# seryrzu/centroFlye

Hardware: NVIDIA B200
Metric: k-mer recruitment read-bases/s (higher is better)
Workload: dtype u64

## Files before the change

### centroflye_b200/csrc/cfk.cu

```cuda
#include <stdlib.h>
#include <string.h>

#include "cfk_common.cuh"

thread_local char cfk_g_err[512] = "";
long long cfk_g_launches = 0;

namespace {

using cfk::EMPTY;
using cfk::FULL;
using cfk::blocks_for;
using cfk::fail;
using cfk::home_slot;
using cfk::mix64;

__device__ __forceinline__ uint32_t base_at(const uint32_t* __restrict__ packed, int64_t pos) {
  return (__ldg(packed + (pos >> 4)) >> ((pos & 15) << 1)) & 3u;
}

__device__ __forceinline__ int64_t table_upsert(uint64_t* keys, int64_t cap, uint64_t key) {
  int64_t slot = home_slot(mix64(key), cap);
  for (int64_t probes = 0; probes < cap; ++probes) {
    uint64_t cur = ((volatile uint64_t*)keys)[slot];
// ... 1586 lines not shown
    if (incr_total) atomicAdd((unsigned long long*)(counters + 2), (unsigned long long)incr_total);
    if (splits) atomicAdd((unsigned long long*)(counters + 3), (unsigned long long)splits);
  }
}

struct JoinArgs {
  const int64_t* __restrict__ occ_ptr;
  const uint32_t* __restrict__ occ;
  const uint32_t* __restrict__ occ_last;
  const uint32_t* __restrict__ unit_last;
  uint32_t dmin, dmax, min_cov;
  double rel_threshold;
  uint4* edges;
  int64_t max_edges;
  uint8_t* selected;
  int64_t* edge_counter;
};

__device__ __forceinline__ uint32_t join_candidate(bool active, uint4 c, const JoinArgs& J) {
  constexpr uint32_t END = 0xFFFFFFFFu;
  uint32_t dmask = 0;
  uint32_t cnt0 = 0;
  uint64_t all_occ = 0;
  uint32_t ia = 0, ia_end = 0, ib0 = 0, ib_end = 0;
  if (active) {
    ia = (uint32_t)J.occ_ptr[c.x]; ia_end = (uint32_t)J.occ_ptr[c.x + 1];
    ib0 = (uint32_t)J.occ_ptr[c.y]; ib_end = (uint32_t)J.occ_ptr[c.y + 1];
    const uint32_t width = c.w - c.z;
    uint32_t ib = ib0;
    uint32_t bj = ib < ib_end ? __ldg(J.occ + ib) : END;
    for (uint32_t t = ia; t < ia_end; ++t) {
      const uint32_t g = __ldg(J.occ + t);
      const uint32_t rem = (J.occ_last ? __ldg(J.occ_last + t) : __ldg(J.unit_last + g)) - g;
      if (J.dmin > rem) continue;
      const uint32_t lo = g + J.dmin, hi = g + min(J.dmax, rem);
      while (bj < lo) {
        ++ib;
        bj = ib < ib_end ? __ldg(J.occ + ib) : END;
      }
      uint32_t jj = ib, v = bj;
      while (v <= hi) {
        ++all_occ;
        const uint32_t dj = (v - g) - c.z;
        if (dj <= width) dmask |= 1u << dj;
        cnt0 += dj == 0u;
        ++jj;
        v = jj < ib_end ? __ldg(J.occ + jj) : END;
      }
    }
  }
  uint32_t n_cand_d = 0;
  while (__any_sync(FULL, dmask != 0)) {
    bool keep = false;
    uint32_t d = 0, cnt = 0;
    if (dmask) {
      const uint32_t dj = (uint32_t)(__ffs(dmask) - 1);
      d = c.z + dj;
      dmask &= dmask - 1;
      if (dj == 0u) {
        cnt = cnt0;
      } else {
        uint32_t ib = ib0;
        uint32_t bj = ib < ib_end ? __ldg(J.occ + ib) : END;
        for (uint32_t t = ia; t < ia_end; ++t) {
          const uint32_t g = __ldg(J.occ + t);
          const uint32_t rem = (J.occ_last ? __ldg(J.occ_last + t) : __ldg(J.unit_last + g)) - g;
          if (d > rem) continue;
          const uint32_t want = g + d;
          while (bj < want) {
            ++ib;
            bj = ib < ib_end ? __ldg(J.occ + ib) : END;
          }
          cnt += bj == want;
        }
      }
      if (cnt >= J.min_cov) {
        ++n_cand_d;
        keep = ((double)cnt / (double)all_occ) >= J.rel_threshold;
      }
    }
    const int64_t pos = warp_append(keep, J.edge_counter);
    if (keep) {
      if (pos < J.max_edges) J.edges[pos] = make_uint4(c.x, c.y, d, cnt);
      J.selected[c.x] = 1;
      J.selected[c.y] = 1;
    }
  }
  return n_cand_d;
}

constexpr int SK_BITS = CFK_SKETCH_BITS;
constexpr int SK_TBL_BYTES = 1 << SK_BITS;
constexpr uint32_t SK_OFF_MASK = 0x3FFFu;
constexpr uint32_t SK_DUP = 0x8000u;
constexpr uint32_t SK_NULL = SK_DUP | (uint32_t)SK_TBL_BYTES;
constexpr int SK_PAD_BYTES = 128;
constexpr int SK_L2_SLOTS = 256;
constexpr int SK_L2_MAX = 192;
constexpr int SK_Q_SLOTS = 256;
constexpr int SK_WINDOW = 128;
constexpr int SK_WARP_BYTES = SK_TBL_BYTES + SK_PAD_BYTES + SK_L2_SLOTS * 4 + SK_Q_SLOTS * 4;
constexpr int SK_WARPS_FIT = (227 * 1024 - 256) / SK_WARP_BYTES;
constexpr int SK_WARPS = SK_WARPS_FIT > 32 ? 32 : SK_WARPS_FIT;
constexpr uint32_t SK_CAP = (uint32_t)SK_TBL_BYTES / CFK_SKETCH_LOAD_DIV;
constexpr int SK_ND_MAX = 16;
static_assert(SK_BITS >= 10 && SK_BITS <= 13, "codes are 16 bit: offset in bits 0..13 (the null byte sits at 2^SK_BITS), bit 15 = no store");
static_assert(SK_WARPS >= 1, "sketch does not fit shared memory");

__host__ __device__ __forceinline__ int64_t sk_block(int64_t first_entry, int64_t unit) { return (first_entry >> 7) + unit; }
static_assert(SK_WINDOW == 128, "sk_block shifts by 7");

__device__ __forceinline__ uint32_t sk_hash(uint32_t id) { return (id * 0x9E3779B1u) >> (32 - SK_BITS); }

__device__ __forceinline__ uint32_t lds_u8(uint32_t a) {
  uint32_t v;
  asm volatile("ld.shared.u8 %0, [%1];" : "=r"(v) : "r"(a) : "memory");
  return v;
}
__device__ __forceinline__ void sts_u8(uint32_t a, uint32_t v) { asm volatile("st.shared.u8 [%0], %1;" ::"r"(a), "r"(v) : "memory"); }
__device__ __forceinline__ uint32_t atom_cas_shared(uint32_t a, uint32_t cmp, uint32_t val) {
  uint32_t old;
  asm volatile("atom.shared.cas.b32 %0, [%1], %2, %3;" : "=r"(old) : "r"(a), "r"(cmp), "r"(val) : "memory");
  return old;
}

__global__ void __launch_bounds__(256) sketch_codes_kernel(const int64_t* __restrict__ unit_ptr, const uint32_t* __restrict__ ids,
                                                           int64_t n_units, uint2* __restrict__ codes) {
  __shared__ uint32_t bm[8][SK_TBL_BYTES / 32];
  const int lane = threadIdx.x & 31, warp = threadIdx.x >> 5;
  const int64_t u = (int64_t)blockIdx.x * 8 + warp;
  if (u >= n_units) return;
  const int64_t b = unit_ptr[u], e = unit_ptr[u + 1];
  if (b == e) return;
  for (int i = lane; i < SK_TBL_BYTES / 32; i += 32) bm[warp][i] = 0;
  __syncwarp();
  uint2* out = codes + sk_block(b, u) * 32 + lane;
  for (int64_t p0 = b; p0 < e; p0 += SK_WINDOW, out += 32) {
    uint32_t c[4];
#pragma unroll
    for (int j = 0; j < 4; ++j) {
      const int64_t p = p0 + 32 * j + lane;
      c[j] = SK_NULL;
      if (p < e) {
        const uint32_t h = sk_hash(ids[p]);
        const uint32_t old = atomicOr(&bm[warp][h >> 5], 1u << (h & 31u));
        c[j] = h | (((old >> (h & 31u)) & 1u) ? SK_DUP : 0u);
      }
    }
    *out = make_uint2(c[0] | (c[1] << 16), c[2] | (c[3] << 16));
  }
}

__global__ void __launch_bounds__(256) sketch_codes_banked_kernel(const int64_t* __restrict__ unit_ptr,
                                                                  const uint32_t* __restrict__ ids, int64_t n_units,
                                                                  uint2* __restrict__ codes, uint4* __restrict__ perm_ids) {
  __shared__ uint32_t bm[8][SK_TBL_BYTES / 32];
  __shared__ int s_cnt[8][32];
  __shared__ int s_nover[8];
  __shared__ uint16_t s_code[8][SK_WINDOW], s_ocode[8][SK_WINDOW];
  __shared__ uint32_t s_id[8][SK_WINDOW], s_oid[8][SK_WINDOW];
  __shared__ uint8_t s_free[8][SK_WINDOW];
  const int lane = threadIdx.x & 31, warp = threadIdx.x >> 5;
  const uint32_t lt = (1u << lane) - 1u;
  const int64_t u = (int64_t)blockIdx.x * 8 + warp;
  if (u >= n_units) return;
  const int64_t b = unit_ptr[u], e = unit_ptr[u + 1];
  if (b == e) return;
  for (int i = lane; i < SK_TBL_BYTES / 32; i += 32) bm[warp][i] = 0;
  __syncwarp();
  int64_t blk = sk_block(b, u);
  for (int64_t p0 = b; p0 < e; p0 += SK_WINDOW, ++blk) {
    const int n = (int)min((int64_t)SK_WINDOW, e - p0), rows = (n + 31) >> 5;
    s_cnt[warp][lane] = 0;
    if (lane == 0) s_nover[warp] = 0;
#pragma unroll
    for (int j = 0; j < 4; ++j) {
      s_code[warp][4 * lane + j] = (uint16_t)(SK_DUP | (uint32_t)(SK_TBL_BYTES + 4 * lane));
      s_id[warp][4 * lane + j] = 0u;
    }
    __syncwarp();
#pragma unroll
    for (int j = 0; j < 4; ++j) {
      const int q = 32 * j + lane;
      if (q < n) {
        const uint32_t id = ids[p0 + q];
        const uint32_t h = sk_hash(id);
        const uint32_t old = atomicOr(&bm[warp][h >> 5], 1u << (h & 31u));
        const uint16_t code = (uint16_t)(h | (((old >> (h & 31u)) & 1u) ? SK_DUP : 0u));
        const int bank = (int)((h >> 2) & 31u);
        const int r = atomicAdd(&s_cnt[warp][bank], 1);
        if (r < rows) {
          s_code[warp][4 * bank + r] = code;
          s_id[warp][4 * bank + r] = id;
        } else {
          const int o = atomicAdd(&s_nover[warp], 1);
          s_ocode[warp][o] = code;
          s_oid[warp][o] = id;
        }
      }
    }
    __syncwarp();
    const int mine = min(s_cnt[warp][lane], rows);
    int base = 0;
    for (int r = rows - 1; r >= 0; --r) {
      const bool fr = mine <= r;
      const unsigned bal = __ballot_sync(FULL, fr);
      if (fr) s_free[warp][base + __popc(bal & lt)] = (uint8_t)(4 * lane + r);
      base += __popc(bal);
    }
    __syncwarp();
    const int nover = s_nover[warp];
    for (int o = lane; o < nover; o += 32) {
      const int slot = s_free[warp][o];
      s_code[warp][slot] = s_ocode[warp][o];
      s_id[warp][slot] = s_oid[warp][o];
    }
    __syncwarp();
    const uint32_t c0 = s_code[warp][4 * lane], c1 = s_code[warp][4 * lane + 1], c2 = s_code[warp][4 * lane + 2],
                   c3 = s_code[warp][4 * lane + 3];
    codes[blk * 32 + lane] = make_uint2(c0 | (c1 << 16), c2 | (c3 << 16));
    perm_ids[blk * 32 + lane] = make_uint4(s_id[warp][4 * lane], s_id[warp][4 * lane + 1], s_id[warp][4 * lane + 2],
                                           s_id[warp][4 * lane + 3]);
    __syncwarp();
  }
}

struct SketchArgs {
  const int64_t* __restrict__ unit_ptr;
  const uint32_t* __restrict__ ids;
  bool banked;
  const uint2* __restrict__ codes;
  const uint32_t* __restrict__ unit_last;
  const uint32_t* __restrict__ last_a;
  const uint32_t* __restrict__ occ_a;
  int64_t m;
  int64_t n_kmers;
  uint32_t a;
  uint32_t thr;
  uint4* cand;
  int64_t max_cand;
  int64_t* counters;
  struct SketchChunk* chunk;
  bool prefetch;
};

constexpr int SK_CAND_CHUNK = 256;
constexpr uint32_t SK_NO_CAND = 0xFFFFFFFFu;
struct SketchChunk {
  int64_t pos, end, emitted;
};

__device__ __forceinline__ void sk_close_chunk(const SketchArgs& A) {
  const int lane = threadIdx.x & 31;
  for (int64_t q = A.chunk->pos + lane; q < A.chunk->end; q += 32)
    if (q < A.max_cand) A.cand[q] = make_uint4(SK_NO_CAND, 0u, 0u, 0u);
  A.chunk->pos = A.chunk->end;
}

__device__ bool sk_drain(uint32_t l2base, uint32_t qbase, const SketchArgs& A, int qn, int64_t lo_id, int64_t hi_id,
                         int& claims) {
  const int lane = threadIdx.x & 31;
  bool ovf = false;
  __syncwarp();
  for (int base = 0; base < qn; base += 32) {
    const int idx = base + lane;
    if (idx < qn) {
      const uint32_t pos = lds<uint32_t>(qbase + (uint32_t)idx * 4u);
      const uint32_t b = __ldg(A.ids + pos);
      if (b != A.a && (int64_t)b >= lo_id && (int64_t)b < hi_id) {
        const uint32_t key = b + 1u;
        uint32_t slot = (b * 0x85EBCA77u) >> 24;
        static_assert(SK_L2_SLOTS == 256, "slot hash takes the top 8 bits");
        int probes = 0;
        for (; probes < SK_L2_SLOTS; ++probes) {
          const uint32_t old = atom_cas_shared(l2base + slot * 4u, 0u, key);
          if (old == 0u) { ++claims; break; }
          if (old == key) break;
          slot = (slot + 1u) & (uint32_t)(SK_L2_SLOTS - 1);
        }
        if (probes == SK_L2_SLOTS) ovf = true;
      }
    }
  }
  __syncwarp();
  const int total = __reduce_add_sync(FULL, claims);
  return !(__any_sync(FULL, ovf) || total > SK_L2_MAX);
}

struct SketchPre {
  uint32_t up, ue;
  int64_t unit;
};

__device__ __forceinline__ void sk_prefetch_unit(const uint2* codes, uint32_t up, uint32_t ue, uint32_t ub) {
  if (ue <= up) return;
  const uint32_t n_blocks = (ue - up + (uint32_t)SK_WINDOW - 1u) / (uint32_t)SK_WINDOW;
  const char* base = reinterpret_cast<const char*>(codes + (size_t)ub * 32u);
  for (uint32_t b = 0; b < n_blocks && b < 4u; ++b) {
    asm volatile("prefetch.global.L2 [%0];" ::"l"(base + b * 256u));
    asm volatile("prefetch.global.L2 [%0];" ::"l"(base + b * 256u + 128u));
  }
}

__device__ int sketch_pass(uint32_t tbase, const SketchArgs& A, int d0, int nd, int64_t lo_id, int64_t hi_id,
                           const SketchPre* pre = nullptr) {
  const int lane = threadIdx.x & 31;
  const uint32_t lt = (1u << lane) - 1u;
  const uint32_t l2base = tbase + SK_TBL_BYTES + SK_PAD_BYTES, qbase = l2base + SK_L2_SLOTS * 4;
  const uint32_t thr = A.thr;
  uint32_t up = 0, ue = 0, ub = 0;
  unsigned rest = 0;
  int src = 0;
  uint32_t p = 0, e = 0, cb = 0;
  uint2 w = make_uint2(0, 0);
  if (pre != nullptr) {
    up = pre->up;
    ue = pre->ue;
    ub = (uint32_t)sk_block((int64_t)up, pre->unit);
    if (A.prefetch) sk_prefetch_unit(A.codes, up, ue, ub);
    rest = __ballot_sync(FULL, ue > up);
    if (rest) {
      src = __ffs(rest) - 1;
      rest &= rest - 1;
      p = __shfl_sync(FULL, up, src); e = __shfl_sync(FULL, ue, src); cb = __shfl_sync(FULL, ub, src);
      w = __ldg(A.codes + (size_t)cb * 32u + lane);
    }
  }
#pragma unroll 4
  for (int i = lane; i < (SK_TBL_BYTES + SK_PAD_BYTES + SK_L2_SLOTS * 4) / 16; i += 32)
    sts128(tbase + (uint32_t)i * 16u, make_uint4(0, 0, 0, 0));
  __syncwarp();
  int qn = 0, claims = 0;
  const int64_t n_items = A.m * (int64_t)nd;
  for (int64_t i0 = 0; i0 < n_items; i0 += 32) {
    if (pre != nullptr) {
      if (e <= p) continue;
    } else {
      const int64_t it = i0 + lane;
      up = 0; ue = 0; ub = 0;
      if (it < n_items) {
        const int64_t t = (nd == 1) ? it : it / nd;
        const int64_t g = (int64_t)__ldg(A.occ_a + t);
        const int64_t u = g + d0 + (it - t * nd);
        if (u <= last_unit_of(A.unit_last, A.last_a, t, g)) {
          const int64_t p0 = __ldg(A.unit_ptr + u);
          up = (uint32_t)p0;
          ue = (uint32_t)__ldg(A.unit_ptr + u + 1);
          ub = (uint32_t)sk_block(p0, u);
        }
      }
      if (A.prefetch) sk_prefetch_unit(A.codes, up, ue, ub);
      rest = __ballot_sync(FULL, ue > up);
      if (!rest) continue;
      src = __ffs(rest) - 1;
      rest &= rest - 1;
      p = __shfl_sync(FULL, up, src); e = __shfl_sync(FULL, ue, src); cb = __shfl_sync(FULL, ub, src);
      w = __ldg(A.codes + (size_t)cb * 32u + lane);
    }
    for (;;) {
      uint32_t np = p + SK_WINDOW, ne = e, ncb = cb + 1u;
      const bool sw = np >= ne;
      const int nsrc = (__ffs(rest) - 1) & 31;
      const uint32_t sp = __shfl_sync(FULL, up, nsrc), se = __shfl_sync(FULL, ue, nsrc), sb = __shfl_sync(FULL, ub, nsrc);
      const bool more = !sw || rest != 0u;
      np = sw ? sp : np;
      ne = sw ? se : ne;
      ncb = sw ? sb : ncb;
      rest = sw ? (rest & (rest - 1u)) : rest;
      uint2 nw = make_uint2(0, 0);
      if (more) nw = __ldg(A.codes + (size_t)ncb * 32u + lane);
      const uint32_t a0 = tbase + (w.x & SK_OFF_MASK), a1 = tbase + ((w.x >> 16) & SK_OFF_MASK);
      const uint32_t a2 = tbase + (w.y & SK_OFF_MASK), a3 = tbase + ((w.y >> 16) & SK_OFF_MASK);
      const uint32_t o0 = lds_u8(a0), o1 = lds_u8(a1), o2 = lds_u8(a2), o3 = lds_u8(a3);
      if (!(w.x & SK_DUP)) sts_u8(a0, min(o0 + 1u, 255u));
      if ((int32_t)w.x >= 0) sts_u8(a1, min(o1 + 1u, 255u));
      if (!(w.y & SK_DUP)) sts_u8(a2, min(o2 + 1u, 255u));
      if ((int32_t)w.y >= 0) sts_u8(a3, min(o3 + 1u, 255u));
      if (__any_sync(FULL, max(max(o0, o1), max(o2, o3)) >= thr)) {
        const bool hs[4] = {o0 >= thr, o1 >= thr, o2 >= thr, o3 >= thr};
#pragma unroll
        for (int i = 0; i < 4; ++i) {
          const unsigned bal = __ballot_sync(FULL, hs[i]);
          if (hs[i]) sts(qbase + (uint32_t)(qn + __popc(bal & lt)) * 4u, A.banked ? (cb << 7) + 4u * (uint32_t)lane + (uint32_t)i : p + (uint32_t)lane + 32u * i);
          qn += __popc(bal);
        }
        if (qn > SK_Q_SLOTS - SK_WINDOW) {
          if (!sk_drain(l2base, qbase, A, qn, lo_id, hi_id, claims)) return -1;
          qn = 0;
        }
      }
      __syncwarp();
      if (!more) break;
      p = np; e = ne; cb = ncb; w = nw;
    }
  }
  if (!sk_drain(l2base, qbase, A, qn, lo_id, hi_id, claims)) return -1;
  int emitted = 0;
  for (int i = lane; i < SK_L2_SLOTS / 4; i += 32) {
    const uint4 q = lds128(l2base + (uint32_t)i * 16u);
    const uint32_t w[4] = {q.x, q.y, q.z, q.w};
    if (__any_sync(FULL, (q.x | q.y | q.z | q.w) != 0u)) {
#pragma unroll
      for (int j = 0; j < 4; ++j) {
        const bool take = w[j] != 0u;
        const unsigned bal = __ballot_sync(FULL, take);
        if (bal) {
          const int n = __popc(bal);
          if (A.chunk->pos + n > A.chunk->end) {
            sk_close_chunk(A);
            unsigned long long base = 0;
            if (lane == 0) base = atomicAdd((unsigned long long*)A.counters, (unsigned long long)SK_CAND_CHUNK);
            base = __shfl_sync(FULL, base, 0);
            A.chunk->pos = (int64_t)base;
            A.chunk->end = (int64_t)base + SK_CAND_CHUNK;
          }
          const int64_t pos = A.chunk->pos + __popc(bal & lt);
          if (take && pos < A.max_cand) A.cand[pos] = make_uint4(A.a, w[j] - 1u, (uint32_t)d0, (uint32_t)(d0 + nd - 1));
          A.chunk->pos += n;
          A.chunk->emitted += n;
        }
        emitted += take;
      }
    }
  }
  __syncwarp();
  return emitted;
}

__device__ void sketch_source(uint32_t tbase, const SketchArgs& A, int dmin, int dlim, int64_t& splits) {
  const int lane = threadIdx.x & 31;
  int d0 = dmin;
  int nd_force = SK_ND_MAX;
  const bool cached = A.m <= 32;
  int64_t cg = 0, clim = 0;
  uint32_t W0 = 0, W1 = 0, W2 = 0, W3 = 0, W4 = 0;
  auto window_at = [&](int d) -> uint32_t { return lane < A.m ? (uint32_t)__ldg(A.unit_ptr + min(cg + d, clim)) : 0u; };
  if (cached) {
    if (lane < A.m) {
      cg = (int64_t)__ldg(A.occ_a + lane);
      clim = last_unit_of(A.unit_last, A.last_a, lane, cg) + 1;
    }
    W0 = window_at(d0); W1 = window_at(d0 + 1); W2 = window_at(d0 + 2); W3 = window_at(d0 + 3); W4 = window_at(d0 + 4);
  }
  auto advance_d = [&](int by) {
    for (int i = 0; i < by; ++i) {
      ++d0;
      if (cached) {
        W0 = W1; W1 = W2; W2 = W3; W3 = W4;
        W4 = window_at(d0 + 4);
      }
    }
  };
  while (d0 <= dlim) {
    const int nd_max = min(nd_force, dlim - d0 + 1);
    int nd = 0;
    uint32_t tot = 0, first = 0;
    bool stop = false;
    for (int jb = 0; jb < nd_max && !stop; jb += 4) {
      uint32_t c0 = 0, c1 = 0, c2 = 0, c3 = 0;
      if (cached && jb == 0) {
        c0 = W1 - W0; c1 = W2 - W1; c2 = W3 - W2; c3 = W4 - W3;
      } else
      for (int64_t t0 = 0; t0 < A.m; t0 += 32) {
        const int64_t t = t0 + lane;
        if (t < A.m) {
          const int64_t g = (int64_t)__ldg(A.occ_a + t);
          const int64_t lim = last_unit_of(A.unit_last, A.last_a, t, g) + 1;
          const int64_t u = g + d0 + jb;
          const uint32_t p0 = (uint32_t)__ldg(A.unit_ptr + min(u, lim)), p1 = (uint32_t)__ldg(A.unit_ptr + min(u + 1, lim)),
                         p2 = (uint32_t)__ldg(A.unit_ptr + min(u + 2, lim)), p3 = (uint32_t)__ldg(A.unit_ptr + min(u + 3, lim)),
                         p4 = (uint32_t)__ldg(A.unit_ptr + min(u + 4, lim));
          c0 += p1 - p0; c1 += p2 - p1; c2 += p3 - p2; c3 += p4 - p3;
        }
      }
      const uint32_t c[4] = {__reduce_add_sync(FULL, c0), __reduce_add_sync(FULL, c1), __reduce_add_sync(FULL, c2),
                             __reduce_add_sync(FULL, c3)};
      if (jb == 0) first = c[0];
#pragma unroll
      for (int k = 0; k < 4; ++k) {
        if (stop || jb + k >= nd_max) { stop = true; continue; }
        if (c[k] <= SK_CAP && tot <= SK_CAP - c[k]) { tot += c[k]; ++nd; } else stop = true;
      }
    }
    if (nd < 1) { nd = 1; tot = first; }
    if (tot == 0) { advance_d(nd); nd_force = SK_ND_MAX; continue; }
    bool redo = false;
    int64_t lo_id = 0, width = A.n_kmers;
    const SketchPre pre{W0, W1, cg + d0};
    const SketchPre* prep = (cached && nd == 1) ? &pre : nullptr;
    while (lo_id < A.n_kmers) {
      const int64_t hi_id = min(A.n_kmers, lo_id + width);
      const int emitted = sketch_pass(tbase, A, d0, nd, lo_id, hi_id, prep);
      if (emitted < 0) {
        ++splits;
        if (nd > 1) { nd_force = nd >> 1; redo = true; break; }
        width = max((int64_t)1, (hi_id - lo_id) >> 1);
        continue;
      }
      lo_id = hi_id;
      if (emitted < SK_L2_MAX / 2 && width < A.n_kmers) width <<= 1;
    }
    if (redo) continue;
    advance_d(nd);
    nd_force = SK_ND_MAX;
  }
}

__global__ void __launch_bounds__(SK_WARPS * 32, 1)
pair_sketch_kernel(const int64_t* __restrict__ unit_ptr, const uint32_t* __restrict__ ids, const uint2* __restrict__ codes,
                   const uint32_t* __restrict__ perm_ids, const uint32_t* __restrict__ unit_last, const int64_t* __restrict__ occ_ptr,
                   const uint32_t* __restrict__ occ, const uint32_t* __restrict__ occ_last, int64_t n_kmers, int64_t a_begin,
                   int64_t a_end, int32_t a_stride, int32_t min_d, int32_t max_d, uint32_t min_cov, uint4* cand,
                   int64_t max_cand, int64_t* counters, int prefetch) {
  extern __shared__ __align__(16) unsigned char pc_smem[];
  const int lane = threadIdx.x & 31, warp = threadIdx.x >> 5;
  const uint32_t tbase = (uint32_t)__cvta_generic_to_shared(pc_smem) + (uint32_t)warp * SK_WARP_BYTES;
  const int dmin = max(min_d, 1);
  int64_t incr_total = 0, splits = 0;
  SketchChunk chunk{0, 0, 0};
  for (;;) {
    unsigned long long item = 0;
    if (lane == 0) item = atomicAdd((unsigned long long*)(counters + 1), 1ull);
    item = __shfl_sync(FULL, item, 0);
    const int64_t a64 = a_begin + (int64_t)item * a_stride;
    if (a64 >= a_end) break;
    const uint32_t a = (uint32_t)a64;
    const int64_t o0 = occ_ptr[a], m = occ_ptr[a + 1] - o0;
    if (m == 0) continue;
    const uint32_t* occ_a = occ + o0;
    const uint32_t* last_a = occ_last ? occ_last + o0 : nullptr;
    const int dlim = source_scope(unit_ptr, unit_last, occ_a, m, dmin, max_d, min_cov, incr_total, last_a);
    if (dlim < dmin) continue;
    SketchArgs A{unit_ptr, perm_ids ? perm_ids : ids, perm_ids != nullptr, codes, unit_last, last_a, occ_a, m, n_kmers, a, min_cov - 1u, cand,
                 max_cand, counters, &chunk, prefetch != 0};
    sketch_source(tbase, A, dmin, dlim, splits);
  }
  {
    SketchArgs A{};
    A.cand = cand;
    A.max_cand = max_cand;
    A.chunk = &chunk;
    sk_close_chunk(A);
  }
  if (lane == 0) {
    if (chunk.emitted) atomicAdd((unsigned long long*)(counters + 4), (unsigned long long)chunk.emitted);
    if (incr_total) atomicAdd((unsigned long long*)(counters + 2), (unsigned long long)incr_total);
    if (splits) atomicAdd((unsigned long long*)(counters + 3), (unsigned long long)splits);
  }
}

__global__ void pair_join_kernel(const uint4* __restrict__ cand, int64_t n_cand, const int64_t* __restrict__ occ_ptr,
                                 const uint32_t* __restrict__ occ, const uint32_t* __restrict__ occ_last,
                                 const uint32_t* __restrict__ unit_last, int32_t min_d, int32_t max_d, uint32_t min_cov,
                                 double rel_threshold, uint4* edges, int64_t max_edges, uint8_t* selected, int64_t* counters) {
  const int64_t i = (int64_t)blockIdx.x * blockDim.x + threadIdx.x;
  const JoinArgs J{occ_ptr, occ, occ_last, unit_last, (uint32_t)max(min_d, 1), (uint32_t)max(max_d, 0), min_cov, rel_threshold,
                   edges, max_edges, selected, counters};
  uint4 c = make_uint4(0xFFFFFFFFu, 0, 0, 0);
  if (i < n_cand) c = cand[i];
  uint32_t n_cand_d = join_candidate(c.x != 0xFFFFFFFFu, c, J);
  for (int o = 16; o >= 1; o >>= 1) n_cand_d += __shfl_xor_sync(FULL, n_cand_d, o);
  if ((threadIdx.x & 31) == 0 && n_cand_d) atomicAdd((unsigned long long*)(counters + 2), (unsigned long long)n_cand_d);
}

__global__ void flag_indices_kernel(const uint8_t* __restrict__ flags, int64_t n, uint32_t* out, int64_t* counters) {
  const int64_t i = (int64_t)blockIdx.x * blockDim.x + threadIdx.x;
  bool take = i < n && flags[i] != 0;
  int64_t pos = warp_append(take, counters);
  if (take) out[pos] = (uint32_t)i;
}


}

extern "C" {

int cfk_abi_version(void) { return 1; }
const char* cfk_last_error(void) { return cfk_g_err; }
int cfk_pair_table_bytes_per_warp(void) { return PC_TBL_BYTES; }
int cfk_pair_warps_per_block(void) { return PC_WARPS; }
int64_t cfk_launch_count(void) { return (int64_t)__atomic_load_n(&cfk_g_launches, __ATOMIC_RELAXED); }

int cfk_table_init(uint64_t* table, int64_t cap, cfk_stream_t stream) {
  if (cap < 1) return fail(CFK_ERR_INVALID, "cfk_table_init: cap < 1");
  table_init_kernel<<<(unsigned)blocks_for(cap, 256), 256, 0, (cudaStream_t)stream>>>(table, cap);
  CFK_CHECK_LAUNCH("table_init_kernel", 1);
  return CFK_OK;
}

int cfk_docfreq_count(const uint32_t* packed, const int64_t* read_off, const int64_t* read_len, const int32_t* order,
                      int64_t n_reads, int k, uint64_t* table, int64_t cap, int64_t* counters, int32_t n_blocks,
                      cfk_stream_t stream) {
  if (k < 1 || k > 31) return fail(CFK_ERR_INVALID, "cfk_docfreq_count: k must be in [1, 31]");
  if (cap < 1 || n_reads < 0 || n_blocks < 1) return fail(CFK_ERR_INVALID, "cfk_docfreq_count: bad sizes");
  if (n_reads == 0) return CFK_OK;
  static unsigned long long attr_done = 0;
  const int smem = (DF_SET_SLOTS + DF_TILE_WORDS) * 4;
  {
    cudaError_t e = cfk::ensure_dynamic_smem(docfreq_kernel, smem, &attr_done);
    if (e != cudaSuccess) return fail(CFK_ERR_CUDA, "cfk_docfreq_count: cudaFuncSetAttribute", e);
  }
  docfreq_kernel<<<(unsigned)n_blocks, DF_THREADS, smem, (cudaStream_t)stream>>>(packed, read_off, read_len, order, n_reads,
                                                                               k, table, cap, counters);
  CFK_CHECK_LAUNCH("docfreq_kernel", 1);
  return CFK_OK;
}

int cfk_docfreq_plan(const int64_t* read_len, const int32_t* order, int64_t n_reads, int k, int32_t* n_pass,
                     cfk_stream_t stream) {
  if (k < 1 || k > 31) return fail(CFK_ERR_INVALID, "cfk_docfreq_plan: k must be in [1, 31]");
  if (n_reads < 0) return fail(CFK_ERR_INVALID, "cfk_docfreq_plan: bad sizes");
  if (n_reads == 0) return CFK_OK;
  docfreq_plan_kernel<<<(unsigned)blocks_for(n_reads, 256), 256, 0, (cudaStream_t)stream>>>(read_len, order, n_reads, k, n_pass);
  CFK_CHECK_LAUNCH("docfreq_plan_kernel", 1);
  return CFK_OK;
}

int cfk_docfreq_count_resident(const uint32_t* packed, const int64_t* read_off, const int64_t* read_len,
                               const int32_t* order, const int64_t* item_ptr, int64_t n_reads, int k, uint64_t* table,
                               int64_t cap, int64_t* counters, int32_t n_blocks, cfk_stream_t stream) {
  if (k < 1 || k > 31) return fail(CFK_ERR_INVALID, "cfk_docfreq_count_resident: k must be in [1, 31]");
  if (cap < 1 || n_reads < 0 || n_blocks < 1) return fail(CFK_ERR_INVALID, "cfk_docfreq_count_resident: bad sizes");
  if (n_reads == 0) return CFK_OK;
  static unsigned long long attr_done = 0;
  const int smem = DF3_SMEM_WORDS * 4;
  {
    cudaError_t e = cfk::ensure_dynamic_smem(docfreq_resident_kernel, smem, &attr_done);
    if (e != cudaSuccess) return fail(CFK_ERR_CUDA, "cfk_docfreq_count_resident: cudaFuncSetAttribute", e);
  }
  docfreq_resident_kernel<<<(unsigned)n_blocks * DF3_BLOCKS_PER_SM, DF3_THREADS, smem, (cudaStream_t)stream>>>(
      packed, read_off, read_len, order, item_ptr, n_reads, k, table, cap, counters);
  CFK_CHECK_LAUNCH("docfreq_resident_kernel", 1);
  return CFK_OK;
}

int cfk_kmer_count_total(const uint32_t* packed, const int64_t* read_off, const int64_t* read_len, const int32_t* tile_read,
                         const int64_t* tile_start, int64_t n_tiles, int k, uint64_t* table, int64_t cap, int64_t* counters,
                         cfk_stream_t stream) {
  if (k < 1 || k > 31) return fail(CFK_ERR_INVALID, "cfk_kmer_count_total: k must be in [1, 31]");
  if (cap < 1 || n_tiles < 0 || n_tiles >= (1ll << 31)) return fail(CFK_ERR_INVALID, "cfk_kmer_count_total: bad sizes");
  if (n_tiles == 0) return CFK_OK;
  kmer_count_kernel<false><<<(unsigned)n_tiles, KC_THREADS, 0, (cudaStream_t)stream>>>(packed, read_off, read_len, tile_read,
                                                                                     tile_start, k, table, cap, counters);
  CFK_CHECK_LAUNCH("kmer_count_kernel", 1);
  return CFK_OK;
}

int cfk_kmer_count_canonical(const uint32_t* packed, const int64_t* read_off, const int64_t* read_len, const int32_t* tile_read,
                             const int64_t* tile_start, int64_t n_tiles, int k, uint64_t* table, int64_t cap,
                             int64_t* counters, cfk_stream_t stream) {
  if (k < 1 || k > 31) return fail(CFK_ERR_INVALID, "cfk_kmer_count_canonical: k must be in [1, 31]");
  if (cap < 1 || n_tiles < 0 || n_tiles >= (1ll << 31)) return fail(CFK_ERR_INVALID, "cfk_kmer_count_canonical: bad sizes");
  if (n_tiles == 0) return CFK_OK;
  kmer_count_kernel<true><<<(unsigned)n_tiles, KC_THREADS, 0, (cudaStream_t)stream>>>(packed, read_off, read_len, tile_read,
                                                                                    tile_start, k, table, cap, counters);
  CFK_CHECK_LAUNCH("kmer_count_kernel", 1);
  return CFK_OK;
}

int cfk_kmer_count_tile(void) { return KC_TILE; }

int cfk_kmer_position_keys(const uint32_t* packed, int64_t n_bases, int k, int pos_bits, uint64_t* keys, cfk_stream_t stream) {
  if (k < 1 || k > 31) return fail(CFK_ERR_INVALID, "cfk_kmer_position_keys: k must be in [1, 31]");
  if (pos_bits < 1 || 2 * k + pos_bits > 63 || n_bases < 0 || n_bases >= (1ll << pos_bits) || n_bases >= (1ll << 32))
    return fail(CFK_ERR_INVALID, "cfk_kmer_position_keys: need n_bases < 2^pos_bits and 2k + pos_bits <= 63");
  const int64_t n = n_bases - k + 1;
  if (n <= 0) return CFK_OK;
  kmer_position_keys_kernel<<<(unsigned)blocks_for(n, 256), 256, 0, (cudaStream_t)stream>>>(packed, n, k, pos_bits, keys);
  CFK_CHECK_LAUNCH("kmer_position_keys_kernel", 1);
  return CFK_OK;
}

int cfk_adjacent_gaps(const uint64_t* keys, int64_t n, int pos_bits, uint32_t* gaps, cfk_stream_t stream) {
  if (n < 0 || pos_bits < 1 || pos_bits > 62) return fail(CFK_ERR_INVALID, "cfk_adjacent_gaps: bad sizes");
  if (n == 0) return CFK_OK;
  adjacent_gaps_kernel<<<(unsigned)blocks_for(n, 256), 256, 0, (cudaStream_t)stream>>>(keys, n, pos_bits, gaps);
  CFK_CHECK_LAUNCH("adjacent_gaps_kernel", 1);
  return CFK_OK;
}

int cfk_table_merge(const uint64_t* keys, const uint32_t* nreads, const uint32_t* nmulti, int64_t n, uint64_t* table,
                    int64_t cap, int64_t* counters, cfk_stream_t stream) {
  if (n < 0 || cap < 1) return fail(CFK_ERR_INVALID, "cfk_table_merge: bad sizes");
  if (n == 0) return CFK_OK;
  table_merge_kernel<<<(unsigned)blocks_for(n, 256), 256, 0, (cudaStream_t)stream>>>(keys, nreads, nmulti, n, table, cap,
                                                                                      counters);
  CFK_CHECK_LAUNCH("table_merge_kernel", 1);
  return CFK_OK;
}

int cfk_table_lookup(const uint64_t* table, int64_t cap, const uint64_t* keys, int64_t n, uint32_t* out_nreads,
                     uint32_t* out_nmulti, cfk_stream_t stream) {
  if (n < 0 || cap < 1) return fail(CFK_ERR_INVALID, "cfk_table_lookup: bad sizes");
  if (n == 0) return CFK_OK;
  table_lookup_kernel<<<(unsigned)blocks_for(n, 256), 256, 0, (cudaStream_t)stream>>>(table, cap, keys, n, out_nreads, out_nmulti);
  CFK_CHECK_LAUNCH("table_lookup_kernel", 1);
// ... 327 lines not shown
```

Before: 5.805 billion.

## Restructure sketch pass to process per-unit row counts with tail-specialized code

The sketch inner loop now tracks, for each unit, how many 32-position rows remain instead of a start/end pair. Full 4-row blocks go through a tight loop that prefetches the next block, and a final partial block is handled by templated variants that touch only 1–3 rows. This removes shared-memory loads, stores and threshold ballots for rows past the unit end, along with the per-iteration shuffles of end positions. The cost is more branching and code size, plus a serial dependent load inside the inner loop.

```diff
diff --git a/centroflye_b200/csrc/cfk.cu b/centroflye_b200/csrc/cfk.cu
--- a/centroflye_b200/csrc/cfk.cu
+++ b/centroflye_b200/csrc/cfk.cu
@@ -1912,28 +1912,65 @@
   }
 }
 
+template <int K>
+__device__ __forceinline__ bool sk_rows(uint2 w, uint32_t pos0, uint32_t tbase, uint32_t qbase, uint32_t l2base,
+                                        const SketchArgs& A, int64_t lo_id, int64_t hi_id, int& qn, int& claims) {
+  const int lane = threadIdx.x & 31;
+  const uint32_t c[4] = {w.x & 0xFFFFu, w.x >> 16, w.y & 0xFFFFu, w.y >> 16};
+  uint32_t a[K], o[K];
+#pragma unroll
+  for (int i = 0; i < K; ++i) {
+    a[i] = tbase + (c[i] & SK_OFF_MASK);
+    o[i] = lds_u8(a[i]);
+  }
+#pragma unroll
+  for (int i = 0; i < K; ++i)
+    if (!(c[i] & SK_DUP)) sts_u8(a[i], min(o[i] + 1u, 255u));
+  uint32_t mx = o[0];
+#pragma unroll
+  for (int i = 1; i < K; ++i) mx = max(mx, o[i]);
+  if (__any_sync(FULL, mx >= A.thr)) {
+    const uint32_t lt = (1u << lane) - 1u;
+    const uint32_t step = A.banked ? 1u : 32u;
+#pragma unroll
+    for (int i = 0; i < K; ++i) {
+      const bool hs = o[i] >= A.thr;
+      const unsigned bal = __ballot_sync(FULL, hs);
+      if (hs) sts(qbase + (uint32_t)(qn + __popc(bal & lt)) * 4u, pos0 + step * (uint32_t)i);
+      qn += __popc(bal);
+    }
+    if (qn > SK_Q_SLOTS - SK_WINDOW) {
+      if (!sk_drain(l2base, qbase, A, qn, lo_id, hi_id, claims)) return false;
+      qn = 0;
+    }
+  }
+  return true;
+}
+
 __device__ int sketch_pass(uint32_t tbase, const SketchArgs& A, int d0, int nd, int64_t lo_id, int64_t hi_id,
                            const SketchPre* pre = nullptr) {
   const int lane = threadIdx.x & 31;
   const uint32_t lt = (1u << lane) - 1u;
   const uint32_t l2base = tbase + SK_TBL_BYTES + SK_PAD_BYTES, qbase = l2base + SK_L2_SLOTS * 4;
-  const uint32_t thr = A.thr;
-  uint32_t up = 0, ue = 0, ub = 0;
+  const uint2* codes = A.codes + lane;
+  uint32_t up = 0, ur = 0, ub = 0;
   unsigned rest = 0;
   int src = 0;
-  uint32_t p = 0, e = 0, cb = 0;
+  uint32_t p = 0, cb = 0, R = 0;
   uint2 w = make_uint2(0, 0);
   if (pre != nullptr) {
     up = pre->up;
-    ue = pre->ue;
+    ur = (pre->ue - up + 31u) >> 5;
     ub = (uint32_t)sk_block((int64_t)up, pre->unit);
-    if (A.prefetch) sk_prefetch_unit(A.codes, up, ue, ub);
-    rest = __ballot_sync(FULL, ue > up);
+    if (A.prefetch) sk_prefetch_unit(A.codes, up, pre->ue, ub);
+    rest = __ballot_sync(FULL, ur != 0u);
     if (rest) {
       src = __ffs(rest) - 1;
       rest &= rest - 1;
-      p = __shfl_sync(FULL, up, src); e = __shfl_sync(FULL, ue, src); cb = __shfl_sync(FULL, ub, src);
-      w = __ldg(A.codes + (size_t)cb * 32u + lane);
+      p = __shfl_sync(FULL, up, src);
+      R = __shfl_sync(FULL, ur, src);
+      cb = __shfl_sync(FULL, ub, src);
+      w = __ldg(codes + (size_t)cb * 32u);
     }
   }
 #pragma unroll 4
@@ -1944,10 +1981,11 @@
   const int64_t n_items = A.m * (int64_t)nd;
   for (int64_t i0 = 0; i0 < n_items; i0 += 32) {
     if (pre != nullptr) {
-      if (e <= p) continue;
+      if (R == 0u) continue;
     } else {
       const int64_t it = i0 + lane;
-      up = 0; ue = 0; ub = 0;
+      uint32_t ue = 0;
+      up = 0; ub = 0;
       if (it < n_items) {
         const int64_t t = (nd == 1) ? it : it / nd;
         const int64_t g = (int64_t)__ldg(A.occ_a + t);
@@ -1960,48 +1998,41 @@
         }
       }
       if (A.prefetch) sk_prefetch_unit(A.codes, up, ue, ub);
-      rest = __ballot_sync(FULL, ue > up);
+      ur = (ue - up + 31u) >> 5;
+      rest = __ballot_sync(FULL, ur != 0u);
       if (!rest) continue;
       src = __ffs(rest) - 1;
       rest &= rest - 1;
-      p = __shfl_sync(FULL, up, src); e = __shfl_sync(FULL, ue, src); cb = __shfl_sync(FULL, ub, src);
-      w = __ldg(A.codes + (size_t)cb * 32u + lane);
+      p = __shfl_sync(FULL, up, src);
+      R = __shfl_sync(FULL, ur, src);
+      cb = __shfl_sync(FULL, ub, src);
+      w = __ldg(codes + (size_t)cb * 32u);
     }
     for (;;) {
-      uint32_t np = p + SK_WINDOW, ne = e, ncb = cb + 1u;
-      const bool sw = np >= ne;
       const int nsrc = (__ffs(rest) - 1) & 31;
-      const uint32_t sp = __shfl_sync(FULL, up, nsrc), se = __shfl_sync(FULL, ue, nsrc), sb = __shfl_sync(FULL, ub, nsrc);
-      const bool more = !sw || rest != 0u;
-      np = sw ? sp : np;
-      ne = sw ? se : ne;
-      ncb = sw ? sb : ncb;
-      rest = sw ? (rest & (rest - 1u)) : rest;
-      uint2 nw = make_uint2(0, 0);
-      if (more) nw = __ldg(A.codes + (size_t)ncb * 32u + lane);
-      const uint32_t a0 = tbase + (w.x & SK_OFF_MASK), a1 = tbase + ((w.x >> 16) & SK_OFF_MASK);
-      const uint32_t a2 = tbase + (w.y & SK_OFF_MASK), a3 = tbase + ((w.y >> 16) & SK_OFF_MASK);
-      const uint32_t o0 = lds_u8(a0), o1 = lds_u8(a1), o2 = lds_u8(a2), o3 = lds_u8(a3);
-      if (!(w.x & SK_DUP)) sts_u8(a0, min(o0 + 1u, 255u));
-      if ((int32_t)w.x >= 0) sts_u8(a1, min(o1 + 1u, 255u));
-      if (!(w.y & SK_DUP)) sts_u8(a2, min(o2 + 1u, 255u));
-      if ((int32_t)w.y >= 0) sts_u8(a3, min(o3 + 1u, 255u));
-      if (__any_sync(FULL, max(max(o0, o1), max(o2, o3)) >= thr)) {
-        const bool hs[4] = {o0 >= thr, o1 >= thr, o2 >= thr, o3 >= thr};
-#pragma unroll
-        for (int i = 0; i < 4; ++i) {
-          const unsigned bal = __ballot_sync(FULL, hs[i]);
-          if (hs[i]) sts(qbase + (uint32_t)(qn + __popc(bal & lt)) * 4u, A.banked ? (cb << 7) + 4u * (uint32_t)lane + (uint32_t)i : p + (uint32_t)lane + 32u * i);
-          qn += __popc(bal);
-        }
-        if (qn > SK_Q_SLOTS - SK_WINDOW) {
-          if (!sk_drain(l2base, qbase, A, qn, lo_id, hi_id, claims)) return -1;
-          qn = 0;
-        }
-      }
+      const uint32_t np = __shfl_sync(FULL, up, nsrc), nR = __shfl_sync(FULL, ur, nsrc), ncb = __shfl_sync(FULL, ub, nsrc);
+      const bool more = rest != 0u;
+      rest &= rest - 1u;
+      const uint2 nw = __ldg(codes + (size_t)(more ? ncb : cb) * 32u);
+      for (; R > 4u; R -= 4u) {
+        const uint2 x = __ldg(codes + ((size_t)cb + 1u) * 32u);
+        if (!sk_rows<4>(w, A.banked ? (cb << 7) + 4u * (uint32_t)lane : p + (uint32_t)lane, tbase, qbase, l2base, A, lo_id,
+                        hi_id, qn, claims))
+          return -1;
+        w = x;
+        ++cb;
+        p += SK_WINDOW;
+      }
+      const uint32_t pos0 = A.banked ? (cb << 7) + 4u * (uint32_t)lane : p + (uint32_t)lane;
+      bool ok;
+      if (R == 4u) ok = sk_rows<4>(w, pos0, tbase, qbase, l2base, A, lo_id, hi_id, qn, claims);
+      else if (R == 3u) ok = sk_rows<3>(w, pos0, tbase, qbase, l2base, A, lo_id, hi_id, qn, claims);
+      else if (R == 2u) ok = sk_rows<2>(w, pos0, tbase, qbase, l2base, A, lo_id, hi_id, qn, claims);
+      else ok = sk_rows<1>(w, pos0, tbase, qbase, l2base, A, lo_id, hi_id, qn, claims);
+      if (!ok) return -1;
       __syncwarp();
       if (!more) break;
-      p = np; e = ne; cb = ncb; w = nw;
+      p = np; R = nR; cb = ncb; w = nw;
     }
   }
   if (!sk_drain(l2base, qbase, A, qn, lo_id, hi_id, claims)) return -1;
```

Result: no change. 5.819 billion, median of 6 (+0.2%).
